# boolsi/boolsi

Measured on AMD Instinct MI355X. Metric: node-state-updates/s, higher is better.
Workload: dtype u32

## Files before the change

### boolsi_amd/csrc/bsx_api.cpp

```cpp
#include <hip/hip_runtime.h>

#include <algorithm>
#include <cstdio>
#include <cstring>
#include <string>

#include "bsx_engine.h"
#include "bsx_host.h"
#include "bsx_lane_lower.h"
#include "bsx_wide_lower.h"

using namespace bsx;

namespace {
thread_local std::string g_create_error;
}

extern "C" const char* bsx_status_string(int status) {
    switch (status) {
        case BSX_OK: return "ok";
        case BSX_ERR_INVALID: return "invalid argument";
        case BSX_ERR_NO_DEVICE: return "no gfx950 device";
        case BSX_ERR_HIP: return "HIP error";
        case BSX_ERR_UNSUPPORTED: return "unsupported network size";
// ... 149 lines not shown
    HIPCHK(h, h->d_wide_desc.upload(L.wdesc));
    HIPCHK(h, h->d_wide_preds.upload(L.wpreds));
    HIPCHK(h, h->d_wide_tt.upload(L.wtt));

    h->n_nodes = n_nodes;
    h->w64 = (n_nodes + 63) / 64;
    h->net.n_nodes = n_nodes;
    h->net.nw = nw;
    h->net.k_mux = k_mux;
    h->net.n_chunks = L.n_chunks;
    h->net.lut_words = (uint32_t)L.lut.size();
    h->net.n_wide = L.n_wide;
    h->net.lut = h->d_lut.p;
    h->net.masks = h->d_masks.p;
    h->net.wide_desc = h->d_wide_desc.p;
    h->net.wide_preds = h->d_wide_preds.p;
    h->net.wide_tt = h->d_wide_tt.p;

    h->cache_lds_slots = L.cache_lds_slots;
    h->lut_mode = L.lut_mode;
    h->shmem = L.shmem;
    h->shmem_attract = L.shmem_attract;
    HIPCHK(h, configure_attract((int)nw, (int)k_mux, h->lut_mode, h->shmem_attract));
    HIPCHK(h, configure_attract_fast((int)nw, (int)k_mux, h->lut_mode, h->shmem_attract, &h->lean_blocks_per_cu));
    h->cache_stride = L.cache_stride;
    {
        const size_t pool_max = h->shmem + (size_t)L.cache_lds_slots * L.cache_stride + 32 + pool_extra_bytes(nw);
        const size_t pool_min = h->shmem + (size_t)64 * L.cache_stride + 32 + pool_extra_bytes(nw);
        h->pool_ok = pool_min <= 160 * 1024 - 1024;
        int blocks = 0;
        if (h->pool_ok) HIPCHK(h, configure_attract_pool((int)nw, (int)k_mux, h->lut_mode, std::min<size_t>(pool_max, 160 * 1024 - 1024), &blocks));
    }
    if (h->knobs.debug) std::fprintf(stderr, "[bsx] network: nw %u k_mux %u lut mode %d (0 L2 bytes, 1 LDS bytes, 2 LDS nibbles) shmem %zu attract shmem %zu lean blocks/CU %d\n", nw, k_mux, (int)h->lut_mode, h->shmem, h->shmem_attract, h->lean_blocks_per_cu);
    HIPCHK(h, configure_target((int)nw, (int)k_mux, h->lut_mode, target_shmem(h->shmem, kTargetHistBins)));
    HIPCHK(h, configure_simulate((int)nw, (int)k_mux, h->lut_mode, h->shmem));
    HIPCHK(h, configure_profile((int)nw, (int)k_mux, h->lut_mode, h->shmem));
    h->have_net = true;
    return BSX_OK;
}

extern "C" int bsx_set_problem_space(bsx_handle h, const uint64_t* origin_state_words,
                                     const uint32_t* any_nodes, uint32_t n_any,
                                     const bsx_fixed* fixed, uint32_t n_fixed,
                                     const bsx_fixed_var* fixed_var, uint32_t n_fixed_var,
                                     const bsx_pert* sched, uint32_t n_sched,
                                     const bsx_pert_var* pert_var, uint32_t n_pert_var) {
    if (!h) return BSX_ERR_INVALID;
    if (!h->have_net) return fail(h, BSX_ERR_STATE, "bsx_set_problem_space before bsx_set_network");
    if (!origin_state_words) return fail(h, BSX_ERR_INVALID, "origin state is null");
    if (n_pert_var > BSX_MAX_PERT_VARIATIONS) return fail(h, BSX_ERR_UNSUPPORTED, "more than BSX_MAX_PERT_VARIATIONS perturbation variations");
    if (n_any > h->n_nodes) return fail(h, BSX_ERR_INVALID, "more 'any' nodes than nodes");
    wide_release_sample(h);
    if (h->wide)
        return wide_set_problem_space(h, origin_state_words, any_nodes, n_any, fixed, n_fixed, fixed_var, n_fixed_var,
                                      sched, n_sched, pert_var, n_pert_var);
    HIPCHK(h, hipSetDevice(h->device));
    h->have_space = false;
    LaneSpace S;
    if (const LowerStatus s = lane_lower_space(h->n_nodes, h->net.nw, h->w64, origin_state_words, any_nodes, n_any, fixed, n_fixed,
                                               fixed_var, n_fixed_var, sched, n_sched, pert_var, n_pert_var, S))
        return fail(h, s.status, s.msg);
    {
        SampleInputs& in = h->inputs;
        in.origin.assign(origin_state_words, origin_state_words + h->w64);
        in.any_nodes.assign(any_nodes, any_nodes + n_any);
        in.fixed.assign(fixed, fixed + n_fixed);
        in.fixed_var.assign(fixed_var, fixed_var + n_fixed_var);
        in.sched.assign(sched, sched + n_sched);
        in.pert_var.assign(pert_var, pert_var + n_pert_var);
    }
    h->model.sched = S.sched;
    h->model.any = S.any;
    h->model.fv = S.fv;
    HIPCHK(h, h->d_any.upload(S.any));
    HIPCHK(h, h->d_fv.upload(S.fv));
    HIPCHK(h, h->d_pv.upload(S.pv));
    HIPCHK(h, h->d_set.upload(S.set));
    HIPCHK(h, h->d_clr.upload(S.clr));
    HIPCHK(h, hipMemset(h->d_cc_journal.p, 0, sizeof(CycleRecord) * kCycleJournalCap));
    HIPCHK(h, hipMemset(h->d_cc_claims.p, 0, sizeof(unsigned int) * kCycleClaimSlots));
    HIPCHK(h, hipMemset(h->d_cc_count.p, 0, sizeof(unsigned int)));
    h->fast_ok = true;
    h->plan = PlanState();
    h->life_valid = 0;
    h->image_n = ~size_t(0);
    h->h_journal.clear();
    h->journal_stale = true;
    h->fast_steps = 0;
    h->fast_calibrated = false;
    h->variant_count = S.variant_count;
    h->variant_count_saturated = S.variant_count_saturated;
    h->tp_max = S.tp_max;
    DevSpace sp = S.sp;
    sp.any_nodes = h->d_any.p;
    sp.fv = h->d_fv.p;
    sp.pv = h->d_pv.p;
    sp.sched_set = h->d_set.p;
    sp.sched_clr = h->d_clr.p;
    h->sp = sp;
    h->have_space = true;
    return BSX_OK;
}
```

### boolsi_amd/csrc/bsx_cascade.cpp

```cpp
#include <cmath>
#include <cstdio>
#include <cstring>

#include "bsx_attract_host.h"

using namespace bsx;

namespace {
constexpr uint64_t kUnresCap = 1ull << 16;
constexpr uint64_t kNearBytes = 1ull << 32;
}

namespace bsx {

static int mirror_slots_for(bsx_handle h, uint32_t* slots_out) {
    const uint64_t entries = (h->cube_mirror ? 2 : 1) * h->journal_states;
    uint32_t slots = 64;
    while (slots < 2 * entries && slots < h->cache_lds_slots) slots *= 2;
    const size_t fixed = h->shmem + 32 + pool_extra_bytes(h->net.nw);
    while (slots < 4 * entries && slots < h->cache_lds_slots && fixed + (size_t)2 * slots * h->cache_stride <= 80 * 1024) slots *= 2;
    h->mirror_slots = *slots_out = std::min(slots, h->cache_lds_slots);
    if (h->knobs.debug) std::fprintf(stderr, "[bsx] mirror: %llu cycle states cached, %u slots\n", (unsigned long long)h->journal_states, *slots_out);
    return BSX_OK;
}
// ... 52 lines not shown
    if (need & ~h->life_valid) {
        LifetimeParams L{};
        L.net = h->net;
        for (int w = 0; w < kMaxW32; ++w) { L.fixmask[w] = h->sp.fixmask[w]; L.fixval[w] = h->sp.fixval[w]; L.base[w] = c.base[w]; L.free_mask[w] = c.free_mask[w]; }
        L.n_digits = r;
        for (uint32_t q = 0; q < r; ++q) L.node[q] = h->model.any[c.rel[q]];
        HIPCHK(h, h->d_life.reserve(64));
        HIPCHK(h, hipMemsetAsync(h->d_life.p, 0, 64 * sizeof(uint32_t), h->stream));
        L.out = h->d_life.p;
        HIPCHK(h, launch_digit_lifetimes((int)h->net.nw, (int)h->net.k_mux, h->lut_mode, h->shmem, h->stream, L));
        uint32_t measured[64];
        HIPCHK(h, hipMemcpyAsync(measured, h->d_life.p, sizeof(measured), hipMemcpyDeviceToHost, h->stream));
        HIPCHK(h, hipStreamSynchronize(h->stream));
        for (uint32_t q = 0; q < r; ++q) h->life_cache[c.rel[q]] = measured[q];
        h->life_valid |= need;
    }
    uint32_t life[64];
    for (uint32_t q = 0; q < r; ++q) life[q] = h->life_cache[c.rel[q]];
    std::vector<uint32_t> idx(r);
    for (uint32_t q = 0; q < r; ++q) idx[q] = q;
    std::stable_sort(idx.begin(), idx.end(), [&](uint32_t x, uint32_t y) { return life[x] < life[y]; });
    std::vector<uint32_t> rel(r);
    for (uint32_t q = 0; q < r; ++q) rel[q] = c.rel[idx[q]];
    c.rel = rel;
    return BSX_OK;
}

int fetch_counters(bsx_handle h, uint32_t n_blocks) {
    if (!h->knobs.spin_wait) {
        HIPCHK(h, hipMemcpyAsync(h->h_ctr, h->d_ctr, sizeof(Counters) * n_blocks, hipMemcpyDeviceToHost, h->stream));
        HIPCHK(h, hipStreamSynchronize(h->stream));
        return BSX_OK;
    }
    const uint32_t seq = ++h->flag_seq ? h->flag_seq : ++h->flag_seq;
    HIPCHK(h, launch_publish(reinterpret_cast<const uint32_t*>(h->d_ctr), reinterpret_cast<uint32_t*>(h->h_ctr),
                             (uint32_t)(sizeof(Counters) / 4 * n_blocks), const_cast<uint32_t*>(h->h_flag), seq,
                             reinterpret_cast<unsigned int*>(reinterpret_cast<char*>(h->d_level) + kPublishTicketOffset), h->stream));
    uint32_t polls = 0;
    while (__atomic_load_n(h->h_flag, __ATOMIC_ACQUIRE) != seq) {
        __builtin_ia32_pause();
        if ((++polls & 0xFFFFu) == 0) {
            const hipError_t q = hipStreamQuery(h->stream);
            if (q == hipSuccess) {
                if (__atomic_load_n(h->h_flag, __ATOMIC_ACQUIRE) == seq) break;
                return fail(h, BSX_ERR_HIP, "the cascade finished without publishing its counters");
            }
            if (q != hipErrorNotReady) { h->error = std::string("hipStreamQuery: ") + hipGetErrorString(q); return BSX_ERR_HIP; }
        }
    }
    return BSX_OK;
}

CascadeShape cascade_shape(bsx_handle h, const CascadeEnv& env) {
    CascadeShape sh{};
    sh.tp = h->sp.tp_origin;
    sh.cap_rel = env.max_t == BSX_T_INF ? BSX_T_INF : env.max_t - sh.tp;
    sh.cap_rel32 = (sh.cap_rel == BSX_T_INF || sh.cap_rel >= (kStepLimit / 4)) ? 0xFFFFFFFFu : (uint32_t)sh.cap_rel;
    sh.fast_steps = (uint32_t)std::min<uint64_t>((uint64_t)sh.cap_rel32 + 1, std::min<uint32_t>(kFastStepsMax, std::max(192u, 4 * h->fast_steps)));
    uint32_t max_depth = h->knobs.cube_depth ? h->knobs.cube_depth : 8;
    if (h->plan.cube_depth_cap) max_depth = std::min(max_depth, h->plan.cube_depth_cap);
    if (sh.tp) max_depth = (uint32_t)std::min<uint64_t>(max_depth, sh.tp);
    sh.max_depth = std::max(1u, std::min(max_depth, sh.fast_steps > 1 ? sh.fast_steps - 1 : 1u));
    sh.forced_depth = h->knobs.cube_depth != 0;
    return sh;
}

struct ChainLevel {
    uint32_t depth = 0, k_bits = 0, r_here = 0, unit_shift = 0;
    bool per_parent = false;
    Cube cube;
};
struct Chain {
    Cube c1;
    std::vector<uint64_t> rel_mask;
    std::vector<ChainLevel> lv;
    uint32_t top = 1;
    uint32_t ctr_base = 0;
    uint32_t desc_base = 0;
    uint32_t index = 0;
    dim3 top_grid;
};
enum ChainVerdict { kChainOk = 0, kChainLower = 1, kChainRepeat = 2, kChainGiveUp = 3 };

int plan_chain(bsx_handle h, const CascadeShape& sh, const Cube& c1, uint32_t top, Chain& ch) {
    ch.c1 = c1;
    ch.lv.clear();
    cube_levels(h->model, h->sp, c1, sh.max_depth, ch.rel_mask);
    ch.top = top ? std::min<uint32_t>(top, (uint32_t)ch.rel_mask.size()) : choose_top(h->plan, sh, ch.rel_mask, sh.max_depth);
    if (__builtin_popcountll(ch.rel_mask[ch.top - 1]) > 47) return BSX_OK;
    ch.lv.resize(ch.top);
    for (uint32_t i = 0; i < ch.top; ++i) {
        const uint32_t d = ch.top - i;
        const uint64_t here = ch.rel_mask[d - 1], digits = i == 0 ? here : here & ~ch.rel_mask[d];
        ChainLevel& l = ch.lv[i];
        l.depth = d;
        l.r_here = (uint32_t)__builtin_popcountll(here);
        l.cube = c1;
        l.cube.rel.clear();
        for (uint32_t j = 0; j < c1.a; ++j) if ((digits >> j) & 1ull) l.cube.rel.push_back(j);
        if (i == 0) if (int rc = order_cube_digits(h, l.cube)) return rc;
        plan_cube(h->model, h->sp, l.cube);
        l.k_bits = (uint32_t)l.cube.rel.size();
        l.unit_shift = c1.n_free - l.r_here;
    }
    return BSX_OK;
}

struct ChainBatch {
    uint32_t slots = 0;
    size_t shmem = 0;
    Launch full{};
    uint64_t seg_cap = 0;
    uint32_t n_side = 0;
    bool two_tops = false;
};

int prepare_batch(bsx_handle h, const CascadeEnv& env, const std::vector<Chain*>& chains, ChainBatch& B, bool& ok) {
    ok = false;
    const uint32_t nw = h->net.nw, rec_words = nw + 3;
    h->cube_mirror = true;
    const int rc_m = lean_mirror_slots(h, &B.slots, &env.tot);
    h->cube_mirror = false;
    if (rc_m) return rc_m;
    uint64_t states = 0;
    for (const CycleRecord& jr : h->h_journal) states += jr.length;
    if (h->h_journal.size() > (size_t)kTagAcc + kLdsAcc || 4 * states > h->cache_lds_slots) return BSX_OK;
    B.shmem = h->shmem + (size_t)B.slots * h->cache_stride + 32 + pool_extra_bytes(nw);
    B.full = plan_persistent(h, ~0ull >> 8, B.shmem);
    uint32_t top_bits = 16, blocks = 0;
    bool lists = false;
    for (const Chain* ch : chains) {
        if (ch->lv.empty()) continue;
        top_bits = std::max(top_bits, ch->lv[0].k_bits);
        lists = lists || ch->top > 1;
        blocks += ch->top;
    }
    const uint64_t list_cap = std::min<uint64_t>(kNearBytes / (4 * (nw + 1)), 1ull << top_bits);
    B.seg_cap = h->knobs.cube_near_cap ? h->knobs.cube_near_cap : std::max<uint64_t>(64, list_cap / B.full.grid.x);
    uint32_t n_lists = 0;
    for (const Chain* ch : chains) n_lists += (!ch->lv.empty() && ch->top > 1) ? 1u : 0u;
    B.n_side = std::min<uint32_t>(n_lists, (uint32_t)h->knobs.cube_streams);
    if (B.n_side < 2) B.n_side = lists ? 1 : 0;
    for (uint32_t sl = 0; sl < B.n_side; ++sl) {
        HIPCHK(h, h->d_near_seg[sl].reserve((size_t)B.full.grid.x * B.seg_cap * (nw + 1)));
        for (auto& list : h->d_near_list[sl]) HIPCHK(h, list.reserve((size_t)B.full.grid.x * B.seg_cap * (nw + 1)));
        if (B.n_side > 1 && !h->side[sl]) HIPCHK(h, hipStreamCreateWithFlags(&h->side[sl], hipStreamNonBlocking));
    }
    HIPCHK(h, h->d_unres.reserve((size_t)std::max(blocks, 1u) * kUnresCap * rec_words));
    B.two_tops = h->knobs.cube_top_streams == 2 && B.n_side > 1;
    if (B.two_tops && !h->top2) {
        HIPCHK(h, hipStreamCreateWithFlags(&h->top2, hipStreamNonBlocking));
        HIPCHK(h, hipEventCreateWithFlags(&h->ev_top2, hipEventDisableTiming));
    }
    ok = true;
    return BSX_OK;
}

int enqueue_chain(bsx_handle h, const CascadeEnv& env, const CascadeShape& sh, const ChainBatch& B, Chain& ch, uint32_t slot,
                  std::vector<hipEvent_t>& slot_busy) {
    const uint32_t nw = h->net.nw, rec_words = nw + 3;
    const bool side = B.n_side > 1 && ch.top > 1;
    hipStream_t const main_st = (B.two_tops && (ch.index & 1u)) ? h->top2 : h->stream, tail_st = side ? h->side[slot] : h->stream;
    hipEvent_t* const ev = h->ev_chain.data() + 3 * (size_t)ch.index;
    if (side && slot_busy[slot]) HIPCHK(h, hipStreamWaitEvent(main_st, slot_busy[slot], 0));
    AttractParams Q0 = env.P;
    Q0.cc.lds_slots = B.slots;
    Q0.merge = 3;
    Q0.fast_steps = sh.fast_steps;
    Q0.per_problem = nullptr;
    Q0.offsets = nullptr;
    Q0.states = nullptr;
// ... 131 lines not shown
    uint32_t blocks = 0, n_live = 0;
    for (Chain* ch : chains) {
        if (ch->lv.empty()) continue;
        ch->ctr_base = blocks;
        ch->desc_base = blocks + n_live;
        ch->index = n_live++;
        blocks += ch->top;
    }
    if (!n_live) return BSX_OK;
    if (blocks > kMaxChainBlocks || n_live > kMaxChains) return fail(h, BSX_ERR_INVALID, "internal: too many chains in one batch");
    while (h->ev_chain.size() < 3 * (size_t)n_live) {
        hipEvent_t e = nullptr;
        HIPCHK(h, hipEventCreate(&e));
        h->ev_chain.push_back(e);
    }
    if (!h->h_leaf) HIPCHK(h, hipHostMalloc((void**)&h->h_leaf, sizeof(LeafProgram) * kMaxChains, hipHostMallocDefault));
    HIPCHK(h, h->d_leaf.reserve(kMaxChains));
    const double pt0 = now_ms();
    HIPCHK(h, hipMemsetAsync(h->d_level, 0, kLevelDescBytes + sizeof(Counters) * blocks, h->stream));
    HIPCHK(h, hipEventRecord(h->ev0, h->stream));
    {
        std::vector<hipEvent_t> slot_busy(std::max(1u, B.n_side), nullptr);
        uint32_t n_listing = 0;
        for (Chain* ch : chains) {
            if (ch->lv.empty()) continue;
            const uint32_t slot = (B.n_side > 1 && ch->top > 1) ? n_listing++ % B.n_side : 0u;
            if (int rc = enqueue_chain(h, env, sh, B, *ch, slot, slot_busy)) return rc;
            if (B.two_tops && ch->index == 0) HIPCHK(h, hipStreamWaitEvent(h->top2, h->ev_chain[0], 0));
        }
        if (B.two_tops) {
            HIPCHK(h, hipEventRecord(h->ev_top2, h->top2));
            HIPCHK(h, hipStreamWaitEvent(h->stream, h->ev_top2, 0));
        }
        for (hipEvent_t e : slot_busy) if (e) HIPCHK(h, hipStreamWaitEvent(h->stream, e, 0));
    }
    HIPCHK(h, hipEventRecord(h->ev1, h->stream));
    const double pt1 = now_ms();
    if (int rc = fetch_counters(h, blocks)) return rc;
    ++tot.syncs;
    const double pt2 = now_ms();
    float ms = 0.f;
    if (hipEventElapsedTime(&ms, h->ev0, h->ev1) != hipSuccess) {
        HIPCHK(h, hipEventSynchronize(h->ev1));
        HIPCHK(h, hipEventElapsedTime(&ms, h->ev0, h->ev1));
    }
    tot.prof[1] += pt1 - pt0; tot.prof[2] += pt2 - pt1; tot.prof[3] += ms;
    tot.kernel_ms += ms;
    h->ctr_seen.assign(h->h_ctr, h->h_ctr + blocks);
    for (Chain* ch : chains) {
        if (ch->lv.empty()) continue;
        float ms_top = 0.f;
        HIPCHK(h, hipEventElapsedTime(&ms_top, h->ev_chain[3 * ch->index], h->ev_chain[3 * ch->index + 1]));
        tot.launches += ch->top;
        tot.dominant_ms += ms_top;
        tot.dominant_exec += h->h_ctr[ch->ctr_base].steps_exec;
        ++tot.dominant_launches;
        if (h->knobs.debug) {
            std::string line;
            double sum = ms_top * 1e3;
            char buf[96];
            std::snprintf(buf, sizeof buf, "d%u %.0f", ch->top, ms_top * 1e3);
            line += buf;
            for (uint32_t i = 1; i < ch->top; ++i) {
                const Counters& c = h->h_ctr[ch->ctr_base + i];
                const double us = (c.t_last && c.t_first_not) ? (double)(c.t_last - ~c.t_first_not) / h->wall_clock_khz * 1e3 : 0.0;
                sum += us;
                std::snprintf(buf, sizeof buf, " | d%u %.0f", ch->top - i, us);
                line += buf;
            }
            std::fprintf(stderr, "[bsx] chain %u: estimated %.0f us, took %.0f us (%s)\n", ch->index, chain_cost_us(h->plan, ch->rel_mask, ch->top), sum, line.c_str());
        }
        for (uint32_t i = 1; i < ch->top; ++i) {
            const Counters& c = h->h_ctr[ch->ctr_base + i];
            if (!c.t_last || !c.t_first_not) continue;
            tot.lower_ms += (double)(c.t_last - ~c.t_first_not) / h->wall_clock_khz;
            tot.lower_exec += c.steps_exec;
            ++tot.lower_launches;
        }
    }
    ++tot.launches;
    return BSX_OK;
}

int run_cubes(bsx_handle h, const CascadeEnv& env, const std::vector<Cube>& cubes, bool& collapsed) {
    collapsed = false;
    Totals& tot = env.tot;
    const CascadeShape sh = cascade_shape(h, env);
    std::vector<uint32_t> top(cubes.size(), 0);
    std::vector<char> done(cubes.size(), 0);
    Totals part;
    const CascadeEnv env_part{env.P, env.max_t, env.max_len, part, env.d_log};
    auto book_device_time = [&]() {
        tot.steps_exec += part.steps_exec; tot.kernel_ms += part.kernel_ms; tot.launches += part.launches;
        tot.dominant_ms += part.dominant_ms; tot.dominant_exec += part.dominant_exec; tot.dominant_launches += part.dominant_launches;
        tot.lower_ms += part.lower_ms; tot.lower_exec += part.lower_exec; tot.lower_launches += part.lower_launches;
        tot.syncs += part.syncs; tot.limit_hits += part.limit_hits;
        for (int s = 0; s < 6; ++s) tot.prof[s] += part.prof[s];
    };
    for (int attempt = 0; attempt < 32; ++attempt) {
        const double pt_plan = now_ms();
        std::vector<Chain> chains;
        std::vector<size_t> who;
        chains.reserve(cubes.size());
        for (size_t i = 0; i < cubes.size(); ++i) {
            if (done[i]) continue;
            chains.emplace_back();
            who.push_back(i);
            if (int rc = plan_chain(h, sh, cubes[i], top[i], chains.back())) return rc;
            if (chains.back().lv.empty()) { book_device_time(); return BSX_OK; }
        }
        if (chains.empty()) break;
        std::vector<Chain*> ptrs;
        uint32_t blocks = 0;
        for (Chain& ch : chains) { ptrs.push_back(&ch); blocks += ch.top; }
        if (blocks > kMaxChainBlocks || chains.size() > kMaxChains) { book_device_time(); return BSX_OK; }
        if (ptrs.size() > 2 && h->knobs.cube_order_tails) {
            auto tail_us = [&](const Chain* ch) {
                const double top_us = kLevelOverheadUs + std::ldexp(1.0, __builtin_popcountll(ch->rel_mask[ch->top - 1])) * (ch->top + 0.3) / 4.5e5;
                return chain_cost_us(h->plan, ch->rel_mask, ch->top) - top_us;
            };
            std::vector<std::pair<double, Chain*>> keyed;
            for (Chain* ch : ptrs) keyed.emplace_back(-tail_us(ch), ch);
            std::stable_sort(keyed.begin(), keyed.end(), [](const std::pair<double, Chain*>& a, const std::pair<double, Chain*>& b) { return a.first < b.first; });
            for (size_t i = 0; i < ptrs.size(); ++i) ptrs[i] = keyed[i].second;
        }
        ChainBatch B;
        bool ok = false;
        if (int rc = prepare_batch(h, env_part, ptrs, B, ok)) return rc;
        if (!ok) { book_device_time(); return BSX_OK; }
        part.prof[0] += now_ms() - pt_plan;
        if (int rc = run_batch(h, env_part, sh, B, ptrs)) return rc;
        bool repeat = false;
        const double pt_eval = now_ms();
        for (size_t q = 0; q < chains.size(); ++q) {
            MergedTable pass_table;
            u128 pass_none = 0, pass_ref = 0;
            int verdict = kChainOk;
            uint32_t lower_to = 0;
            if (int rc = evaluate_chain(h, env_part, sh, chains[q], pass_table, pass_none, pass_ref, verdict, lower_to)) return rc;
            if (verdict == kChainOk) {
                fold_table(part.merged, pass_table);
                part.n_none += pass_none;
                part.steps_ref += pass_ref;
                done[who[q]] = 1;
            } else if (verdict == kChainLower && lower_to >= 1) {
                if (h->knobs.debug)
                    std::fprintf(stderr, "[bsx] chain %u: a list overflowed, again from depth %u\n", chains[q].index, lower_to);
                top[who[q]] = lower_to;
                if (cubes.size() == 1) h->plan.cube_depth_cap = lower_to;
            } else if (verdict == kChainRepeat) {
                repeat = true;
            } else {
                book_device_time();
                return BSX_OK;
            }
        }
        part.prof[5] += now_ms() - pt_eval;
        if (repeat) {
            unsigned int known = 0;
            HIPCHK(h, hipMemcpy(&known, h->d_cc_count.p, sizeof(known), hipMemcpyDeviceToHost));
            ++part.syncs;
            if (known <= h->h_journal.size()) { book_device_time(); return BSX_OK; }
        }
    }
    book_device_time();
    for (char d : done) if (!d) return BSX_OK;
    fold_table(tot.merged, part.merged);
    tot.n_none += part.n_none;
    tot.steps_ref += part.steps_ref;
    collapsed = true;
    return BSX_OK;
}

}

namespace bsx {

int run_block(bsx_handle h, const CascadeEnv& env, uint64_t d_lo, uint32_t a_bits, bool& collapsed) {
    collapsed = false;
    const CascadeShape sh = cascade_shape(h, env);
    const bool forced = h->knobs.cube_split == 1;
    if (h->knobs.cube_split != 0 && sh.tp == 0 && (a_bits >= kSplitMinBits || forced)) {
        std::vector<std::pair<uint64_t, uint64_t>>& tree = h->plan.split_cache[a_bits];
        auto estimate = [&]() {
            double est = 0;
            for (const auto& l : tree) est += cube_cost_us(h->model, h->sp, h->plan, sh, d_lo, a_bits, l.first, l.second);
            return est;
        };
        double experience = 0;
        for (uint32_t d = 0; d <= kMaxCubeLevels; ++d) experience += h->plan.near_seen[0][d][0];
        auto grow = [&]() {
            const double t0 = now_ms();
            std::vector<SplitLeaf> fresh;
            plan_split(h->model, h->sp, h->plan, sh, d_lo, a_bits, forced, fresh);
            tree.clear();
            for (const SplitLeaf& l : fresh) tree.emplace_back(l.mask, l.vals);
            h->plan.split_learned[a_bits] = experience;
            if (h->knobs.debug)
                std::fprintf(stderr, "[bsx] split tree for blocks of 2^%u: %zu leaves, planned in %.2f ms (list fractions from %.3g classes seen)\n", a_bits,
                             tree.size(), now_ms() - t0, experience);
        };
        const double pt_est = now_ms();
        const double whole = cube_cost_us(h->model, h->sp, h->plan, sh, d_lo, a_bits, 0, 0);
        bool use = false;
        if (tree.empty() || experience > 64.0 * (h->plan.split_learned[a_bits] + 1024.0)) { grow(); use = tree.size() > 1; }
        else if (tree.size() > 1) {
            use = forced || estimate() < 0.8 * whole;
            if (!use && a_bits >= 60 && h->plan.split_regrown[a_bits] < 2) { ++h->plan.split_regrown[a_bits]; grow(); use = tree.size() > 1; }
        }
        env.tot.prof[4] += now_ms() - pt_est;
        if (use) {
            std::vector<Cube> cubes(tree.size());
            bool eligible = true;
            for (size_t i = 0; i < tree.size() && eligible; ++i) {
                build_cube(h->model, h->sp, d_lo, a_bits, cubes[i], nullptr, tree[i].first, tree[i].second);
                if (!cubes[i].ok || cubes[i].rel.size() + 2 > cubes[i].n_free) eligible = false;
            }
            if (eligible) {
                if (int rc = run_cubes(h, env, cubes, collapsed)) return rc;
                if (collapsed) return BSX_OK;
            }
        }
    }
    Cube c;
    build_cube(h->model, h->sp, d_lo, a_bits, c);
    if (c.ok && c.rel.size() + 2 <= a_bits) return run_cubes(h, env, std::vector<Cube>{c}, collapsed);
    return BSX_OK;
}

}
```

### boolsi_amd/csrc/bsx_cube_plan.cpp

```cpp
#include "bsx_cube_plan.h"

#include <algorithm>
#include <cmath>
#include <cstring>
#include <utility>

namespace bsx {

void build_cube(const HostModel& m, const DevSpace& sp, uint64_t d_lo, uint32_t a, Cube& c, const uint32_t* fixmask, uint64_t fix_mask, uint64_t fix_vals) {
    if (!fixmask) fixmask = sp.fixmask;
    const uint32_t n = m.n_nodes, nw = m.nw;
    c.d_lo = d_lo; c.a = a; c.rel.clear(); c.ok = false;
    const uint64_t low = a >= 64 ? ~0ull : (1ull << a) - 1ull;
    c.fix_mask = fix_mask & low; c.fix_vals = fix_vals & c.fix_mask;
    c.free_digits = low & ~c.fix_mask;
    c.n_free = (uint32_t)__builtin_popcountll(c.free_digits);
    uint32_t base[kMaxW32];
    for (int w = 0; w < kMaxW32; ++w) { base[w] = sp.origin[w]; c.umask[w] = 0; c.free_mask[w] = 0; }
    std::vector<char> is_free(n, 0), relevant(n, 0);
    for (uint32_t j = 0; j < sp.n_any; ++j) {
        const uint32_t node = m.any[j];
        if (j < a && ((c.free_digits >> j) & 1ull)) { is_free[node] = 1; c.free_mask[node >> 5] |= 1u << (node & 31); }
        else if (j < a ? ((c.fix_vals >> j) & 1ull) != 0 : ((d_lo >> j) & 1ull) != 0) base[node >> 5] |= 1u << (node & 31);
    }
// ... 80 lines not shown
            do {
                const uint32_t idx = fixed_idx | x;
                seen |= 1u << ((tt >> idx) & 1ull);
                for (uint32_t j = 0; j < k; ++j)
                    if (((var_slots >> j) & 1u) && (((tt >> idx) ^ (tt >> (idx ^ (1u << j)))) & 1ull)) sens |= 1u << j;
                x = (x - var_slots) & var_slots;
            } while (x);
            if (seen != 3u) { nval[i] = seen >> 1; continue; }
            nval[i] = 2;
            for (uint32_t j = 0; j < k; ++j) if ((sens >> j) & 1u) ndep[i] |= dep[preds[j]];
        }
        for (size_t e = 0; e + 2 < m.sched.size(); e += 3)
            if (m.sched[e] == d) { nval[m.sched[e + 1]] = (uint8_t)m.sched[e + 2]; ndep[m.sched[e + 1]] = 0; }
        all = 0;
        for (uint32_t i = 0; i < n; ++i) all |= ndep[i];
        out.push_back(all);
        val.swap(nval);
        dep.swap(ndep);
    }
}

bool build_leaf_program(const HostModel& m, const DevSpace& sp, const std::vector<uint32_t>& added_digits, LeafProgram& L) {
    const uint32_t n = m.n_nodes;
    if (added_digits.empty() || added_digits.size() > kLeafMaxBits) return false;
    static_assert(kLeafMaxBits <= 16 && kLeafMaxDeps <= 64, "digit_node[], the free rules' 64-bit masks (bsx_leaf.h)");
    std::memset(&L, 0, sizeof(L));
    L.kb = (uint32_t)added_digits.size();
    std::vector<int> digit_of(n, -1);
    for (uint32_t q = 0; q < L.kb; ++q) {
        const uint32_t node = m.any[added_digits[q]];
        digit_of[node] = (int)q;
        L.added[node >> 5] |= 1u << (node & 31);
    }
    std::vector<uint32_t> dep_nodes, dep_digits;
    uint32_t entangled = 0;
    for (uint32_t i = 0; i < n; ++i) {
        uint32_t reads = 0;
        const uint32_t k = m.pred_offsets[i + 1] - m.pred_offsets[i];
        const uint32_t* preds = m.pred_idx.data() + m.pred_offsets[i];
        if (!((sp.fixmask[i >> 5] >> (i & 31)) & 1u))
            for (uint32_t j = 0; j < k; ++j) if (digit_of[preds[j]] >= 0) reads |= 1u << digit_of[preds[j]];
        if (!reads) { L.indep[i >> 5] |= 1u << (i & 31); continue; }
        if (k > kLeafMaxK || dep_nodes.size() == kLeafMaxDeps) return false;
        dep_nodes.push_back(i);
        dep_digits.push_back(reads);
        if (reads & (reads - 1u)) entangled |= reads;
    }
    std::vector<uint32_t> number(L.kb, 0);
    L.m = (uint32_t)__builtin_popcount(entangled);
    for (uint32_t q = 0, e = 0, f = L.m; q < L.kb; ++q) {
        number[q] = ((entangled >> q) & 1u) ? e++ : f++;
        L.digit_node[number[q]] = (uint16_t)m.any[added_digits[q]];
    }
    std::vector<std::pair<uint32_t, uint32_t>> order;
    for (uint32_t r = 0; r < dep_nodes.size(); ++r)
        order.emplace_back((dep_digits[r] & entangled) ? 0u : 1u + number[(uint32_t)__builtin_ctz(dep_digits[r])], r);
    std::sort(order.begin(), order.end());
    for (const auto& o : order) {
        const uint32_t i = dep_nodes[o.second];
        const uint32_t k = m.pred_offsets[i + 1] - m.pred_offsets[i];
        const uint32_t* preds = m.pred_idx.data() + m.pred_offsets[i];
        LeafDep& d = L.dep[L.n_dep++];
        d.node = (uint16_t)i;
        d.k = (uint16_t)(o.first ? k | ((o.first - 1u) << 8) : k);
        (o.first ? L.n_free : L.n_enum)++;
        for (uint32_t j = 0; j < k; ++j)
            d.in[j] = digit_of[preds[j]] >= 0 ? (uint16_t)(0x8000u | number[(uint32_t)digit_of[preds[j]]]) : (uint16_t)preds[j];
        d.tt = (uint32_t)(m.tt0[i] & ((1ull << (1u << k)) - 1ull));
    }
    return true;
}

double near_fraction(const PlanState& ps, uint32_t d, bool is_top) {
    d = std::min<uint32_t>(d, kMaxCubeLevels);
    const auto& seen = ps.near_seen[is_top ? 0 : 1];
    if (seen[d][0] >= 1024.0) return std::min(1.0, seen[d][1] / seen[d][0]);
    for (uint32_t off = 1; off <= kMaxCubeLevels; ++off) {
        if (d > off && seen[d - off][0] >= 1024.0) return std::min(1.0, seen[d - off][1] / seen[d - off][0] * std::ldexp(1.0, (int)off));
        if (d + off <= kMaxCubeLevels && seen[d + off][0] >= 1024.0) return std::min(1.0, seen[d + off][1] / seen[d + off][0] * std::ldexp(1.0, -(int)off));
    }
    return is_top ? std::min(1.0, 0.0025 * std::ldexp(1.0, (int)d - 2)) : 0.1;
}

double chain_cost_us(const PlanState& ps, const std::vector<uint64_t>& rel_mask, uint32_t top) {
    int r_above = __builtin_popcountll(rel_mask[top - 1]);
    double n = std::ldexp(1.0, r_above);
    double cost = kLevelOverheadUs + n * (top + 0.3) / 4.5e5;
    for (uint32_t d = top - 1; d >= 1; --d) {
        const double parents = n * near_fraction(ps, d + 1, d + 1 == top);
        if (parents < 1.0) { cost += 5.0 * d; break; }
        const int r_d = __builtin_popcountll(rel_mask[d - 1]), kb = r_d - r_above;
        n = parents * std::ldexp(1.0, kb);
        cost += kLevelOverheadUs + ((d == 1 && kb >= 1 && kb <= (int)kLeafMaxBits) ? n / 1.5e6 + parents / 2.0e4 : n * (d + 0.3) / 4.5e5);
        r_above = r_d;
    }
    return cost;
}

uint32_t choose_top(const PlanState& ps, const CascadeShape& sh, const std::vector<uint64_t>& rel_mask, uint32_t max_depth, double* est_out) {
    uint32_t top = 1;
    double best = 0;
    for (uint32_t d = 1; d <= max_depth && d <= rel_mask.size(); ++d) {
        const double est = sh.forced_depth ? (double)__builtin_popcountll(rel_mask[d - 1]) : chain_cost_us(ps, rel_mask, d);
        if (d == 1 || est < best) { best = est; top = d; }
    }
    if (est_out) *est_out = sh.forced_depth ? chain_cost_us(ps, rel_mask, top) : best;
    return top;
}


double cube_cost_us(const HostModel& m, const DevSpace& sp, const PlanState& ps, const CascadeShape& sh, uint64_t d_lo, uint32_t a_bits,
                    uint64_t mask, uint64_t vals, uint64_t* top_rel) {
    Cube c;
    std::vector<uint64_t> rel_mask;
    build_cube(m, sp, d_lo, a_bits, c, nullptr, mask, vals);
    cube_levels(m, sp, c, sh.max_depth, rel_mask);
    double est = 0;
    const uint32_t top = choose_top(ps, sh, rel_mask, sh.max_depth, &est);
    if (top_rel) *top_rel = rel_mask[top - 1];
    return est;
}

void plan_split(const HostModel& m, const DevSpace& sp, const PlanState& ps, const CascadeShape& sh, uint64_t d_lo, uint32_t a_bits, bool forced,
                std::vector<SplitLeaf>& leaves) {
    leaves.clear();
    const double min_cost_us = 3 * kLevelOverheadUs;
    std::vector<SplitLeaf> todo{{0, 0}};
    while (!todo.empty()) {
        const SplitLeaf nd = todo.back();
        todo.pop_back();
        uint64_t top_rel = 0;
        const double here = cube_cost_us(m, sp, ps, sh, d_lo, a_bits, nd.mask, nd.vals, &top_rel);
        bool split = false;
        if (forced ? leaves.size() + todo.size() + 2 <= 8 : (here > min_cost_us && leaves.size() + todo.size() + 2 <= kMaxChains)) {
            double best = 0;
            int best_digit = -1;
            for (uint64_t left = top_rel; left; left &= left - 1) {
                const int j = __builtin_ctzll(left);
                const double both = cube_cost_us(m, sp, ps, sh, d_lo, a_bits, nd.mask | (1ull << j), nd.vals) +
                                    cube_cost_us(m, sp, ps, sh, d_lo, a_bits, nd.mask | (1ull << j), nd.vals | (1ull << j));
                if (best_digit < 0 || both < best) { best = both; best_digit = j; }
            }
            if (best_digit >= 0 && (forced || best < 0.85 * here)) {
                todo.push_back(SplitLeaf{nd.mask | (1ull << best_digit), nd.vals});
                todo.push_back(SplitLeaf{nd.mask | (1ull << best_digit), nd.vals | (1ull << best_digit)});
                split = true;
            }
        }
        if (!split) leaves.push_back(nd);
    }
}

}
```

### boolsi_amd/csrc/bsx_cube_plan.h

```cpp
#pragma once
#include <cstdint>
#include <vector>

#include "bsx_device.h"
#include "bsx_model.h"

namespace bsx {

constexpr uint32_t kCubeMinBits = 16;
constexpr uint32_t kCubeMaxBits = 63;
constexpr uint32_t kSplitMinBits = 52;
constexpr double kLevelOverheadUs = 22.0;

struct Cube {
    uint64_t d_lo;
    uint32_t a;
    uint64_t fix_mask = 0, fix_vals = 0, free_digits = 0;
    uint32_t n_free = 0;
    std::vector<uint32_t> rel;
    uint32_t base[kMaxW32];
    DevSpace sp;
    uint32_t umask[kMaxW32];
    uint32_t free_mask[kMaxW32];
    bool ok = false;
};
void build_cube(const HostModel& m, const DevSpace& sp, uint64_t d_lo, uint32_t a, Cube& c, const uint32_t* fixmask = nullptr,
                uint64_t fix_mask = 0, uint64_t fix_vals = 0);
void plan_cube(const HostModel& m, const DevSpace& sp, Cube& c);
void cube_levels(const HostModel& m, const DevSpace& sp, const Cube& c, uint32_t max_depth, std::vector<uint64_t>& out);
bool build_leaf_program(const HostModel& m, const DevSpace& sp, const std::vector<uint32_t>& added_digits, LeafProgram& L);

struct CascadeShape {
    uint64_t tp, cap_rel;
    uint32_t cap_rel32, fast_steps, max_depth;
    bool forced_depth;
};

double near_fraction(const PlanState& ps, uint32_t d, bool is_top);
double chain_cost_us(const PlanState& ps, const std::vector<uint64_t>& rel_mask, uint32_t top);
uint32_t choose_top(const PlanState& ps, const CascadeShape& sh, const std::vector<uint64_t>& rel_mask, uint32_t max_depth, double* est_out = nullptr);
double cube_cost_us(const HostModel& m, const DevSpace& sp, const PlanState& ps, const CascadeShape& sh, uint64_t d_lo, uint32_t a_bits,
                    uint64_t mask, uint64_t vals, uint64_t* top_rel = nullptr);

struct SplitLeaf { uint64_t mask, vals; };
void plan_split(const HostModel& m, const DevSpace& sp, const PlanState& ps, const CascadeShape& sh, uint64_t d_lo, uint32_t a_bits, bool forced,
                std::vector<SplitLeaf>& leaves);

}
```

### boolsi_amd/csrc/bsx_knobs.cpp

```cpp
#include "bsx_knobs.h"

#include <algorithm>
#include <cstdlib>

#include "bsx_device.h"
#include "bsx_wide.h"

namespace bsx {

Knobs Knobs::from_env() {
    auto is_set = [](const char* name) { return std::getenv(name) != nullptr; };
    auto starts_with = [](const char* name, char c) { const char* e = std::getenv(name); return e && e[0] == c; };
    auto zero_or_one = [&](const char* name) { return starts_with(name, '0') ? 0 : starts_with(name, '1') ? 1 : -1; };
    Knobs k;
    k.debug = is_set("BSX_DEBUG");
    k.profile = is_set("BSX_PROFILE");
    k.cycle_cache = !starts_with("BSX_CYCLE_CACHE", '0');
    if (const char* e = std::getenv("BSX_CACHE_LDS_KB")) k.cache_lds_kb = std::max<size_t>(1, (size_t)std::atoi(e));
    if (const char* e = std::getenv("BSX_LUT_MODE")) k.lut_mode = std::atoi(e);
    if (const char* e = std::getenv("BSX_LEAN")) k.lean = std::atoi(e) != 0;
    if (const char* e = std::getenv("BSX_MERGE")) k.merge = std::atoi(e);
    k.force_counting = is_set("BSX_FORCE_COUNTING");
    if (const char* e = std::getenv("BSX_SERVICE_LANES")) k.service_lanes = (uint32_t)std::atoi(e);
    if (const char* e = std::getenv("BSX_CHUNK")) k.chunk = (uint32_t)std::max(64, std::atoi(e));
    k.mirror_image = !starts_with("BSX_MIRROR_IMAGE", '0');
    k.spin_wait = !starts_with("BSX_SPIN_WAIT", '0');
    k.fgraph = starts_with("BSX_FGRAPH", '1');
    k.cubes = !starts_with("BSX_CUBES", '0');
    k.cube_order = !starts_with("BSX_CUBE_ORDER", '0');
    k.cube_order_tails = !starts_with("BSX_CUBE_ORDER_TAILS", '0');
    k.cube_lower = !starts_with("BSX_CUBE_LOWER", '0');
    k.cube_leaf = !starts_with("BSX_CUBE_LEAF", '0');
    if (const char* e = std::getenv("BSX_CUBE_DEPTH")) k.cube_depth = (uint32_t)std::max(1, std::min((int)kMaxCubeLevels, std::atoi(e)));
    if (const char* e = std::getenv("BSX_CUBE_NEAR_CAP")) k.cube_near_cap = (uint64_t)std::max(1, std::atoi(e));
    const char* streams = std::getenv("BSX_CUBE_STREAMS");
    k.cube_streams = std::max(1, std::min((int)kSideStreams, streams ? std::atoi(streams) : (int)kSideStreams));
    k.cube_top_streams = starts_with("BSX_CUBE_TOP_STREAMS", '1') ? 1 : 2;
    k.cube_split = zero_or_one("BSX_CUBE_SPLIT");
    k.sliced = zero_or_one("BSX_SLICED");
    k.wide = starts_with("BSX_WIDE", '1');
    k.wide_host_reduce = starts_with("BSX_WIDE_HOST_REDUCE", '1');
    if (const char* e = std::getenv("BSX_WIDE_CHUNK")) if (e[0]) { k.wide_chunk_set = true; k.wide_chunk = std::strtoull(e, nullptr, 10); }
    k.wide_step_limit = kWideStepLimit;
    if (const char* e = std::getenv("BSX_WIDE_STEP_LIMIT")) k.wide_step_limit = std::max(16u, std::min(kWideStepLimit, (uint32_t)std::atoi(e)));
    if (const char* e = std::getenv("BSX_CORR_BATCH_CELLS")) k.corr_batch_cells = std::strtoull(e, nullptr, 10);
    k.trans_step_limit = kStepLimit;
    if (const char* e = std::getenv("BSX_TRANS_STEP_LIMIT")) k.trans_step_limit = std::max(1u, std::min(kStepLimit, (uint32_t)std::atoi(e)));
    if (const char* e = std::getenv("BSX_WTRANS_CHUNK")) k.wtrans_chunk = std::max(1ull, std::strtoull(e, nullptr, 10));
    return k;
}

}
```

### boolsi_amd/csrc/bsx_knobs.h

```cpp
#pragma once
#include <cstdint>

namespace bsx {

struct Knobs {
    bool debug = false;
    bool profile = false;
    bool cycle_cache = true;
    uint64_t cache_lds_kb = 0;
    int lut_mode = -1;
    bool lean = true;
    int merge = 2;
    bool force_counting = false;
    uint32_t service_lanes = 0;
    uint32_t chunk = 0;
    bool mirror_image = true;
    bool spin_wait = true;
    bool fgraph = false;
    bool cubes = true;
    bool cube_order = true;
    bool cube_order_tails = true;
    bool cube_lower = true;
    bool cube_leaf = true;
    uint32_t cube_depth = 0;
    uint64_t cube_near_cap = 0;
    int cube_streams = 0;
    int cube_top_streams = 2;
    int cube_split = -1;
    int sliced = -1;
    bool wide = false;
    bool wide_host_reduce = false;
    bool wide_chunk_set = false;
    uint64_t wide_chunk = 0;
    uint32_t wide_step_limit = 0;
    uint64_t corr_batch_cells = 0;
    uint32_t trans_step_limit = 0;
    uint64_t wtrans_chunk = 0;

    static Knobs from_env();
};

}
```

### boolsi_amd/csrc/bsx_model.h

```cpp
#pragma once
#include <cstdint>
#include <map>
#include <utility>
#include <vector>

#include "bsx_device.h"

namespace bsx {

struct HostModel {
    uint32_t n_nodes = 0, nw = 0;
    std::vector<uint32_t> pred_offsets, pred_idx;
    std::vector<uint64_t> tt0;
    std::vector<uint32_t> sched;
    std::vector<uint32_t> any;
    std::vector<uint32_t> fv;
};

struct PlanState {
    double near_seen[2][kMaxCubeLevels + 1][2] = {};
    uint32_t cube_depth_cap = 0;
    std::map<uint32_t, std::vector<std::pair<uint64_t, uint64_t>>> split_cache;
    std::map<uint32_t, double> split_learned;
    std::map<uint32_t, uint32_t> split_regrown;
};

}
```

Before: 18640 billion.

## Replace fixed planner overheads with fitted cost model and reuse planned cubes

Replaces the hard-coded per-level overhead constants in the cube planner with a CostModel whose floors and rates are fitted per level type. When side streams overlap, tail levels get a lower weight. The planner also keeps each cube's build, level masks and chosen top from the cost estimate and passes them to run_cubes, so cubes are not rebuilt. This is meant to pick better split trees and top depths and to cut host planning time. The fitted constants may mis-plan networks unlike the ones they were fitted on.

```diff
diff --git a/boolsi_amd/csrc/bsx_api.cpp b/boolsi_amd/csrc/bsx_api.cpp
--- a/boolsi_amd/csrc/bsx_api.cpp
+++ b/boolsi_amd/csrc/bsx_api.cpp
@@ -255,6 +255,7 @@
     HIPCHK(h, hipMemset(h->d_cc_count.p, 0, sizeof(unsigned int)));
     h->fast_ok = true;
     h->plan = PlanState();
+    h->plan.cost = h->knobs.plan_cost_model();
     h->life_valid = 0;
     h->image_n = ~size_t(0);
     h->h_journal.clear();
diff --git a/boolsi_amd/csrc/bsx_cascade.cpp b/boolsi_amd/csrc/bsx_cascade.cpp
--- a/boolsi_amd/csrc/bsx_cascade.cpp
+++ b/boolsi_amd/csrc/bsx_cascade.cpp
@@ -158,11 +158,12 @@
 };
 enum ChainVerdict { kChainOk = 0, kChainLower = 1, kChainRepeat = 2, kChainGiveUp = 3 };
 
-int plan_chain(bsx_handle h, const CascadeShape& sh, const Cube& c1, uint32_t top, Chain& ch) {
+int plan_chain(bsx_handle h, const CascadeShape& sh, const PlannedCube& pc, uint32_t top, bool fresh, Chain& ch) {
+    const Cube& c1 = pc.c;
     ch.c1 = c1;
     ch.lv.clear();
-    cube_levels(h->model, h->sp, c1, sh.max_depth, ch.rel_mask);
-    ch.top = top ? std::min<uint32_t>(top, (uint32_t)ch.rel_mask.size()) : choose_top(h->plan, sh, ch.rel_mask, sh.max_depth);
+    ch.rel_mask = pc.rel_mask;
+    ch.top = top ? std::min<uint32_t>(top, (uint32_t)ch.rel_mask.size()) : fresh ? choose_top(h->plan, sh, ch.rel_mask, sh.max_depth) : pc.top;
     if (__builtin_popcountll(ch.rel_mask[ch.top - 1]) > 47) return BSX_OK;
     ch.lv.resize(ch.top);
     for (uint32_t i = 0; i < ch.top; ++i) {
@@ -460,8 +461,9 @@
     return BSX_OK;
 }
 
-int run_cubes(bsx_handle h, const CascadeEnv& env, const std::vector<Cube>& cubes, bool& collapsed) {
+int run_cubes(bsx_handle h, const CascadeEnv& env, const std::vector<PlannedCube>& cubes, bool& collapsed) {
     collapsed = false;
+    if (cubes.empty()) return BSX_OK;
     Totals& tot = env.tot;
     const CascadeShape sh = cascade_shape(h, env);
     std::vector<uint32_t> top(cubes.size(), 0);
@@ -484,7 +486,7 @@
             if (done[i]) continue;
             chains.emplace_back();
             who.push_back(i);
-            if (int rc = plan_chain(h, sh, cubes[i], top[i], chains.back())) return rc;
+            if (int rc = plan_chain(h, sh, cubes[i], top[i], attempt > 0, chains.back())) return rc;
             if (chains.back().lv.empty()) { book_device_time(); return BSX_OK; }
         }
         if (chains.empty()) break;
@@ -494,8 +496,9 @@
         if (blocks > kMaxChainBlocks || chains.size() > kMaxChains) { book_device_time(); return BSX_OK; }
         if (ptrs.size() > 2 && h->knobs.cube_order_tails) {
             auto tail_us = [&](const Chain* ch) {
-                const double top_us = kLevelOverheadUs + std::ldexp(1.0, __builtin_popcountll(ch->rel_mask[ch->top - 1])) * (ch->top + 0.3) / 4.5e5;
-                return chain_cost_us(h->plan, ch->rel_mask, ch->top) - top_us;
+                double top_us = 0, tail = 0;
+                chain_cost_parts(h->plan, ch->rel_mask, ch->top, &top_us, &tail);
+                return tail;
             };
             std::vector<std::pair<double, Chain*>> keyed;
             for (Chain* ch : ptrs) keyed.emplace_back(-tail_us(ch), ch);
@@ -558,11 +561,15 @@
     collapsed = false;
     const CascadeShape sh = cascade_shape(h, env);
     const bool forced = h->knobs.cube_split == 1;
+    PlannedCube unsplit;
+    bool have_unsplit = false;
     if (h->knobs.cube_split != 0 && sh.tp == 0 && (a_bits >= kSplitMinBits || forced)) {
         std::vector<std::pair<uint64_t, uint64_t>>& tree = h->plan.split_cache[a_bits];
+        std::vector<PlannedCube> planned;
         auto estimate = [&]() {
             double est = 0;
-            for (const auto& l : tree) est += cube_cost_us(h->model, h->sp, h->plan, sh, d_lo, a_bits, l.first, l.second);
+            planned.resize(tree.size());
+            for (size_t i = 0; i < tree.size(); ++i) est += plan_cube_cost(h->model, h->sp, h->plan, sh, d_lo, a_bits, tree[i].first, tree[i].second, planned[i]);
             return est;
         };
         double experience = 0;
@@ -579,31 +586,33 @@
                              tree.size(), now_ms() - t0, experience);
         };
         const double pt_est = now_ms();
-        const double whole = cube_cost_us(h->model, h->sp, h->plan, sh, d_lo, a_bits, 0, 0);
+        h->plan.cost = h->knobs.plan_cost_model(true);
+        const double whole = plan_cube_cost(h->model, h->sp, h->plan, sh, d_lo, a_bits, 0, 0, unsplit);
+        have_unsplit = true;
+        h->plan.cost = h->knobs.plan_cost_model(false);
         bool use = false;
-        if (tree.empty() || experience > 64.0 * (h->plan.split_learned[a_bits] + 1024.0)) { grow(); use = tree.size() > 1; }
+        if (tree.empty() || experience > 64.0 * (h->plan.split_learned[a_bits] + 1024.0)) { grow(); use = tree.size() > 1; if (use) estimate(); }
         else if (tree.size() > 1) {
-            use = forced || estimate() < 0.8 * whole;
-            if (!use && a_bits >= 60 && h->plan.split_regrown[a_bits] < 2) { ++h->plan.split_regrown[a_bits]; grow(); use = tree.size() > 1; }
+            const double est = estimate();
+            use = forced || est < 0.8 * whole;
+            if (!use && a_bits >= 60 && h->plan.split_regrown[a_bits] < 2) { ++h->plan.split_regrown[a_bits]; grow(); use = tree.size() > 1; if (use) estimate(); }
         }
         env.tot.prof[4] += now_ms() - pt_est;
         if (use) {
-            std::vector<Cube> cubes(tree.size());
             bool eligible = true;
-            for (size_t i = 0; i < tree.size() && eligible; ++i) {
-                build_cube(h->model, h->sp, d_lo, a_bits, cubes[i], nullptr, tree[i].first, tree[i].second);
-                if (!cubes[i].ok || cubes[i].rel.size() + 2 > cubes[i].n_free) eligible = false;
-            }
+            for (const PlannedCube& pc : planned) if (!pc.c.ok || pc.c.rel.size() + 2 > pc.c.n_free) eligible = false;
             if (eligible) {
-                if (int rc = run_cubes(h, env, cubes, collapsed)) return rc;
+                if (int rc = run_cubes(h, env, planned, collapsed)) return rc;
                 if (collapsed) return BSX_OK;
             }
         }
     }
-    Cube c;
-    build_cube(h->model, h->sp, d_lo, a_bits, c);
-    if (c.ok && c.rel.size() + 2 <= a_bits) return run_cubes(h, env, std::vector<Cube>{c}, collapsed);
-    return BSX_OK;
-}
-
-}
+    h->plan.cost = h->knobs.plan_cost_model(true);
+    if (!have_unsplit) build_cube(h->model, h->sp, d_lo, a_bits, unsplit.c);
+    if (!unsplit.c.ok || unsplit.c.rel.size() + 2 > a_bits) return BSX_OK;
+    if (!have_unsplit) plan_cube_cost(h->model, h->sp, h->plan, sh, d_lo, a_bits, 0, 0, unsplit);
+    else unsplit.top = choose_top(h->plan, sh, unsplit.rel_mask, sh.max_depth);
+    return run_cubes(h, env, std::vector<PlannedCube>{unsplit}, collapsed);
+}
+
+}
diff --git a/boolsi_amd/csrc/bsx_cube_plan.cpp b/boolsi_amd/csrc/bsx_cube_plan.cpp
--- a/boolsi_amd/csrc/bsx_cube_plan.cpp
+++ b/boolsi_amd/csrc/bsx_cube_plan.cpp
@@ -186,19 +186,30 @@
     return is_top ? std::min(1.0, 0.0025 * std::ldexp(1.0, (int)d - 2)) : 0.1;
 }
 
-double chain_cost_us(const PlanState& ps, const std::vector<uint64_t>& rel_mask, uint32_t top) {
+double chain_cost_parts(const PlanState& ps, const std::vector<uint64_t>& rel_mask, uint32_t top, double* top_us, double* tail_us) {
+    const CostModel& cm = ps.cost;
     int r_above = __builtin_popcountll(rel_mask[top - 1]);
     double n = std::ldexp(1.0, r_above);
-    double cost = kLevelOverheadUs + n * (top + 0.3) / 4.5e5;
+    const double first = cm.top_floor_us + n * (top + 0.3) / cm.top_rate;
+    double cost = first, tail = 0;
     for (uint32_t d = top - 1; d >= 1; --d) {
         const double parents = n * near_fraction(ps, d + 1, d + 1 == top);
-        if (parents < 1.0) { cost += 5.0 * d; break; }
+        if (parents < 1.0) { cost += cm.tail_weight * (cm.empty_us * d); tail += cm.empty_us * d; break; }
         const int r_d = __builtin_popcountll(rel_mask[d - 1]), kb = r_d - r_above;
         n = parents * std::ldexp(1.0, kb);
-        cost += kLevelOverheadUs + ((d == 1 && kb >= 1 && kb <= (int)kLeafMaxBits) ? n / 1.5e6 + parents / 2.0e4 : n * (d + 0.3) / 4.5e5);
+        const double level = (d == 1 && kb >= 1 && kb <= (int)kLeafMaxBits) ? cm.leaf_floor_us + (n / cm.leaf_child_rate + parents / cm.leaf_parent_rate)
+                                                                            : cm.lower_floor_us + n * (d + 0.3) / cm.lower_rate;
+        cost += cm.tail_weight * level;
+        tail += level;
         r_above = r_d;
     }
+    if (top_us) *top_us = first;
+    if (tail_us) *tail_us = tail;
     return cost;
+}
+
+double chain_cost_us(const PlanState& ps, const std::vector<uint64_t>& rel_mask, uint32_t top) {
+    return chain_cost_parts(ps, rel_mask, top, nullptr, nullptr);
 }
 
 uint32_t choose_top(const PlanState& ps, const CascadeShape& sh, const std::vector<uint64_t>& rel_mask, uint32_t max_depth, double* est_out) {
@@ -215,20 +226,24 @@
 
 double cube_cost_us(const HostModel& m, const DevSpace& sp, const PlanState& ps, const CascadeShape& sh, uint64_t d_lo, uint32_t a_bits,
                     uint64_t mask, uint64_t vals, uint64_t* top_rel) {
-    Cube c;
-    std::vector<uint64_t> rel_mask;
-    build_cube(m, sp, d_lo, a_bits, c, nullptr, mask, vals);
-    cube_levels(m, sp, c, sh.max_depth, rel_mask);
-    double est = 0;
-    const uint32_t top = choose_top(ps, sh, rel_mask, sh.max_depth, &est);
-    if (top_rel) *top_rel = rel_mask[top - 1];
+    PlannedCube pc;
+    const double est = plan_cube_cost(m, sp, ps, sh, d_lo, a_bits, mask, vals, pc);
+    if (top_rel) *top_rel = pc.rel_mask[pc.top - 1];
     return est;
+}
+
+double plan_cube_cost(const HostModel& m, const DevSpace& sp, const PlanState& ps, const CascadeShape& sh, uint64_t d_lo, uint32_t a_bits,
+                      uint64_t mask, uint64_t vals, PlannedCube& out) {
+    build_cube(m, sp, d_lo, a_bits, out.c, nullptr, mask, vals);
+    cube_levels(m, sp, out.c, sh.max_depth, out.rel_mask);
+    out.top = choose_top(ps, sh, out.rel_mask, sh.max_depth, &out.est_us);
+    return out.est_us;
 }
 
 void plan_split(const HostModel& m, const DevSpace& sp, const PlanState& ps, const CascadeShape& sh, uint64_t d_lo, uint32_t a_bits, bool forced,
                 std::vector<SplitLeaf>& leaves) {
     leaves.clear();
-    const double min_cost_us = 3 * kLevelOverheadUs;
+    const double min_cost_us = ps.cost.min_split_floors * ps.cost.lower_floor_us;
     std::vector<SplitLeaf> todo{{0, 0}};
     while (!todo.empty()) {
         const SplitLeaf nd = todo.back();
@@ -245,7 +260,7 @@
                                     cube_cost_us(m, sp, ps, sh, d_lo, a_bits, nd.mask | (1ull << j), nd.vals | (1ull << j));
                 if (best_digit < 0 || both < best) { best = both; best_digit = j; }
             }
-            if (best_digit >= 0 && (forced || best < 0.85 * here)) {
+            if (best_digit >= 0 && (forced || best < ps.cost.split_gain * here)) {
                 todo.push_back(SplitLeaf{nd.mask | (1ull << best_digit), nd.vals});
                 todo.push_back(SplitLeaf{nd.mask | (1ull << best_digit), nd.vals | (1ull << best_digit)});
                 split = true;
diff --git a/boolsi_amd/csrc/bsx_cube_plan.h b/boolsi_amd/csrc/bsx_cube_plan.h
--- a/boolsi_amd/csrc/bsx_cube_plan.h
+++ b/boolsi_amd/csrc/bsx_cube_plan.h
@@ -10,7 +10,6 @@
 constexpr uint32_t kCubeMinBits = 16;
 constexpr uint32_t kCubeMaxBits = 63;
 constexpr uint32_t kSplitMinBits = 52;
-constexpr double kLevelOverheadUs = 22.0;
 
 struct Cube {
     uint64_t d_lo;
@@ -38,9 +37,18 @@
 
 double near_fraction(const PlanState& ps, uint32_t d, bool is_top);
 double chain_cost_us(const PlanState& ps, const std::vector<uint64_t>& rel_mask, uint32_t top);
+double chain_cost_parts(const PlanState& ps, const std::vector<uint64_t>& rel_mask, uint32_t top, double* top_us, double* tail_us);
 uint32_t choose_top(const PlanState& ps, const CascadeShape& sh, const std::vector<uint64_t>& rel_mask, uint32_t max_depth, double* est_out = nullptr);
 double cube_cost_us(const HostModel& m, const DevSpace& sp, const PlanState& ps, const CascadeShape& sh, uint64_t d_lo, uint32_t a_bits,
                     uint64_t mask, uint64_t vals, uint64_t* top_rel = nullptr);
+struct PlannedCube {
+    Cube c;
+    std::vector<uint64_t> rel_mask;
+    uint32_t top = 1;
+    double est_us = 0;
+};
+double plan_cube_cost(const HostModel& m, const DevSpace& sp, const PlanState& ps, const CascadeShape& sh, uint64_t d_lo, uint32_t a_bits,
+                      uint64_t mask, uint64_t vals, PlannedCube& out);
 
 struct SplitLeaf { uint64_t mask, vals; };
 void plan_split(const HostModel& m, const DevSpace& sp, const PlanState& ps, const CascadeShape& sh, uint64_t d_lo, uint32_t a_bits, bool forced,
diff --git a/boolsi_amd/csrc/bsx_knobs.cpp b/boolsi_amd/csrc/bsx_knobs.cpp
--- a/boolsi_amd/csrc/bsx_knobs.cpp
+++ b/boolsi_amd/csrc/bsx_knobs.cpp
@@ -1,6 +1,7 @@
 #include "bsx_knobs.h"
 
 #include <algorithm>
+#include <cstdio>
 #include <cstdlib>
 
 #include "bsx_device.h"
@@ -37,6 +38,16 @@
     k.cube_streams = std::max(1, std::min((int)kSideStreams, streams ? std::atoi(streams) : (int)kSideStreams));
     k.cube_top_streams = starts_with("BSX_CUBE_TOP_STREAMS", '1') ? 1 : 2;
     k.cube_split = zero_or_one("BSX_CUBE_SPLIT");
+    k.plan_model = starts_with("BSX_PLAN_MODEL", '0') ? 0 : 1;
+    if (const char* e = std::getenv("BSX_PLAN_TAIL_WEIGHT")) if (e[0]) k.plan_tail_weight = std::max(0.05, std::min(1.0, std::atof(e)));
+    if (const char* e = std::getenv("BSX_PLAN_COSTS")) {
+        double v[8];
+        if (std::sscanf(e, "%lf,%lf,%lf,%lf,%lf,%lf,%lf,%lf", v, v + 1, v + 2, v + 3, v + 4, v + 5, v + 6, v + 7) == 8 &&
+            std::all_of(v, v + 8, [](double x) { return x > 0; })) {
+            k.plan_costs_set = true;
+            std::copy(v, v + 8, k.plan_costs);
+        }
+    }
     k.sliced = zero_or_one("BSX_SLICED");
     k.wide = starts_with("BSX_WIDE", '1');
     k.wide_host_reduce = starts_with("BSX_WIDE_HOST_REDUCE", '1');
@@ -50,4 +61,16 @@
     return k;
 }
 
+CostModel Knobs::plan_cost_model(bool one_stream) const {
+    if (!plan_model) return CostModel::legacy();
+    const bool overlapped = !one_stream && cube_streams > 1;
+    CostModel cm = CostModel::fitted(overlapped);
+    if (plan_costs_set) {
+        cm.top_floor_us = plan_costs[0]; cm.top_rate = plan_costs[1]; cm.lower_floor_us = plan_costs[2]; cm.lower_rate = plan_costs[3];
+        cm.leaf_floor_us = plan_costs[4]; cm.leaf_parent_rate = plan_costs[5]; cm.leaf_child_rate = plan_costs[6]; cm.empty_us = plan_costs[7];
+    }
+    if (overlapped && plan_tail_weight > 0) cm.tail_weight = plan_tail_weight;
+    return cm;
 }
+
+}
diff --git a/boolsi_amd/csrc/bsx_knobs.h b/boolsi_amd/csrc/bsx_knobs.h
--- a/boolsi_amd/csrc/bsx_knobs.h
+++ b/boolsi_amd/csrc/bsx_knobs.h
@@ -1,5 +1,7 @@
 #pragma once
 #include <cstdint>
+
+#include "bsx_model.h"
 
 namespace bsx {
 
@@ -27,6 +29,10 @@
     int cube_streams = 0;
     int cube_top_streams = 2;
     int cube_split = -1;
+    int plan_model = 1;
+    double plan_tail_weight = 0;
+    bool plan_costs_set = false;
+    double plan_costs[8] = {};
     int sliced = -1;
     bool wide = false;
     bool wide_host_reduce = false;
@@ -38,6 +44,7 @@
     uint64_t wtrans_chunk = 0;
 
     static Knobs from_env();
+    CostModel plan_cost_model(bool one_stream = false) const;
 };
 
 }
diff --git a/boolsi_amd/csrc/bsx_model.h b/boolsi_amd/csrc/bsx_model.h
--- a/boolsi_amd/csrc/bsx_model.h
+++ b/boolsi_amd/csrc/bsx_model.h
@@ -17,7 +17,22 @@
     std::vector<uint32_t> fv;
 };
 
+struct CostModel {
+    double top_floor_us, top_rate;
+    double lower_floor_us, lower_rate;
+    double leaf_floor_us, leaf_parent_rate, leaf_child_rate;
+    double empty_us;
+    double tail_weight;
+    double min_split_floors, split_gain;
+
+    static constexpr CostModel legacy() { return CostModel{22.0, 4.5e5, 22.0, 4.5e5, 22.0, 2.0e4, 1.5e6, 5.0, 1.0, 3.0, 0.85}; }
+    static constexpr CostModel fitted(bool overlapped) {
+        return CostModel{32.6406, 448233.0, 14.0491, 511199.0, 23.9688, 46773.7, 1.36228e7, 5.0, overlapped ? 0.4 : 1.0, 3.0, 0.85};
+    }
+};
+
 struct PlanState {
+    CostModel cost = CostModel::fitted(false);
     double near_seen[2][kMaxCubeLevels + 1][2] = {};
     uint32_t cube_depth_cap = 0;
     std::map<uint32_t, std::vector<std::pair<uint64_t, uint64_t>>> split_cache;
```

After: 15990 billion. 0.858x the previous value.
